# ethz-asl/laser_slam

Hardware: NVIDIA H100
Metric: ICP registrations/s (131072-pt scan vs 524288-pt map, 30 iterations) (higher is better)
Workload: dtype f32

## Files before the change

### laser_slam_b200/csrc/ls_api.cu

```cuda
#include <cerrno>
#include <cmath>
#include <cstdarg>
#include <cstddef>
#include <cstdio>
#include <cstdlib>
#include <cstring>
#include <string>
#include <utility>
#include <vector>

#include "../../include/ls_b200.h"
#include "ls_buffer.cuh"
#include "ls_filters.cuh"
#include "ls_kernels.cuh"
#include "ls_occupancy.cuh"

using namespace ls;

#define LS_VERSION 100

struct Workspace {
  cudaStream_t stream = nullptr;
  cudaEvent_t ev0 = nullptr, ev1 = nullptr, ev2 = nullptr, ev_launch = nullptr;
  Buffer<BuildState> bs;
  Buffer<float4> rd;
  Buffer<int> pos;
  Buffer<float> d2;
  Buffer<float4> vq, vpts;
  Buffer<int> ids;
  Buffer<float> d2_out;
  Buffer<uint32_t> qkey, qperm;
  Buffer<float4> rd_s;
  Buffer<float4> sub_pts, sub_nrm, srt_pts, srt_nrm;
  Buffer<uint32_t> pkey;
  Buffer<Entry> tab1;
  Buffer<uint32_t> cnt1, tab1_cell, qtab_local, qtab_total;
  Buffer<Entry> top;
  Buffer<uint32_t> cnt0;
  Buffer<unsigned long long> pyr, topmask;
  Buffer<uint32_t> qtop_start;
  Buffer<float> T_hist;
  IcpWork* work = nullptr;
  BuildJob* job_host = nullptr;
  BuildJob* job_dev = nullptr;
  IcpProblem hp;
  bool stream_dirty = false;
};

struct ls_ctx {
  int device = 0;
  int sm_count = 0;
  int icp_ctas = 0;
  int icp_ctas_max = 0;
  std::string err;
  uint64_t launches = 0;
  std::vector<Workspace*> ws;
  Buffer<IcpProblem> probs_dev;
  PinnedBuffer<IcpProblem> probs_host;
  Buffer<BuildJob> jobs_dev;
  PinnedBuffer<BuildJob> jobs_host;
  Buffer<IcpWork> work_pool;
  Buffer<IcpResult> results_dev;
  PinnedBuffer<IcpResult> results_host;
  Buffer<float4> reading;
  Buffer<float4> ref_stage, ref_nrm_stage;
  Buffer<float> nrm_raw;
  Buffer<float> T0_dev;
  unsigned char* xbuf = nullptr;
  unsigned char* xpeer[8] = {nullptr, nullptr, nullptr, nullptr, nullptr, nullptr, nullptr, nullptr};
  int shard_rank = 0, shard_count = 1;
  bool xconnected = false;
  unsigned int xflag_base = 0;
  bool pending = false;
  int pending_batch = 0;
  std::vector<int> pending_ws;
  std::vector<int> pending_n;
  std::vector<float> pending_T0;
  std::vector<std::pair<const ls_map*, int>> pending_slots;
  lsf::ChainBuffers chain;
};
constexpr int kMaxBatch = 160;

struct ls_scan_slot {
  Buffer<float4> pts, nrm;
  int n = 0;
  uint64_t id = 0;
  bool used = false;
  cudaEvent_t ready = nullptr;
  bool async = false;
};

constexpr int kStageRing = 16;
struct ls_map {
  ls_ctx* ctx = nullptr;
  int capacity = 0, max_pts = 0;
  uint64_t next_id = 1;
  std::vector<ls_scan_slot> slots;
  cudaStream_t up_stream = nullptr;
  Buffer<float> stage[kStageRing];
  cudaEvent_t stage_free[kStageRing] = {};
  uint64_t n_async = 0;
  PinnedBuffer<float> host_stage[kStageRing];
};

namespace {

int fail(ls_ctx* ctx, int code, const char* fmt, ...) {
  char buf[512];
  va_list ap;
  va_start(ap, fmt);
  vsnprintf(buf, sizeof(buf), fmt, ap);
  va_end(ap);
  if (ctx) ctx->err = buf;
  return code;
}

#define BUSY_CHECK(ctx)                                                                                       \
  do {                                                                                                        \
    if ((ctx)->pending) return fail((ctx), LS_ERR_STATE, "a batch is in flight (ls_icp_register_submap_batch_end first)"); \
  } while (0)

#define CU(call)                                                                                      \
  do {                                                                                                \
    cudaError_t e_ = (call);                                                                          \
    if (e_ != cudaSuccess)                                                                            \
      return fail(ctx, e_ == cudaErrorMemoryAllocation ? LS_ERR_NOMEM : LS_ERR_CUDA, "%s: %s", #call, \
                  cudaGetErrorString(e_));                                                            \
  } while (0)

#define LAUNCH_CHECK()                                                                          \
  do {                                                                                          \
    ++ctx->launches;                                                                            \
    cudaError_t e_ = cudaGetLastError();                                                        \
    if (e_ != cudaSuccess) return fail(ctx, LS_ERR_CUDA, "kernel launch: %s", cudaGetErrorString(e_)); \
  } while (0)

inline int blocks_for(int n, int threads, int cap) {
  int b = (n + threads - 1) / threads;
  if (b < 1) b = 1;
  return b > cap ? cap : b;
}

int grow_failed(ls_ctx* ctx, cudaError_t e, const char* group) {
  return fail(ctx, e == cudaErrorMemoryAllocation ? LS_ERR_NOMEM : LS_ERR_CUDA, "%s: %s", group, cudaGetErrorString(e));
}

int ensure_capacity(ls_ctx* ctx, Workspace* w, int n, int m, int max_cells, int max_iter) {
  cudaError_t e;
  if ((size_t)n > w->rd.capacity()) {
    const size_t c = (size_t)(n + n / 8 + 1024), cv = c * LS_VK;
    if ((e = w->rd.reserve(c, c)) || (e = w->pos.reserve(c, c)) || (e = w->d2.reserve(c, c)) || (e = w->vq.reserve(c, c)) ||
        (e = w->vpts.reserve(cv, cv)) || (e = w->ids.reserve(c, c)) || (e = w->d2_out.reserve(c, c)) ||
        (e = w->qkey.reserve(c, c)) || (e = w->qperm.reserve(c, c)) || (e = w->rd_s.reserve(c, c))) {
      w->rd.reset(), w->pos.reset(), w->d2.reset(), w->vq.reset(), w->vpts.reset(), w->ids.reset(), w->d2_out.reset();
      w->qkey.reset(), w->qperm.reset(), w->rd_s.reset();
      return grow_failed(ctx, e, "reading arrays");
    }
  }
  if ((size_t)m > w->sub_pts.capacity()) {
    const int cap = m + m / 8 + 1024;
    int tcap = cap / 17 + 1024;
    const int tmax = (int)((size_t)1536 * 1024 * 1024 / ((size_t)LS_FB3 * 12));
    if (tcap > tmax) tcap = tmax;
    const size_t c = (size_t)cap, t = (size_t)tcap, tf = t * LS_FB3;
    if ((e = w->sub_pts.reserve(c, c)) || (e = w->sub_nrm.reserve(c, c)) || (e = w->srt_pts.reserve(c, c)) ||
        (e = w->srt_nrm.reserve(c, c)) || (e = w->pkey.reserve(c, c)) || (e = w->tab1.reserve(tf, tf)) ||
        (e = w->cnt1.reserve(tf, tf)) || (e = w->tab1_cell.reserve(t, t)) || (e = w->qtab_local.reserve(tf, tf)) ||
        (e = w->qtab_total.reserve(t, t))) {
      w->sub_pts.reset(), w->sub_nrm.reset(), w->srt_pts.reset(), w->srt_nrm.reset(), w->pkey.reset(), w->tab1.reset();
      w->cnt1.reset(), w->tab1_cell.reset(), w->qtab_local.reset(), w->qtab_total.reset();
      return grow_failed(ctx, e, "sub-map arrays");
    }
    CU(cudaMemsetAsync(w->cnt1.get(), 0, tf * sizeof(uint32_t), w->stream));
    w->stream_dirty = true;
  }
  if ((size_t)max_cells + 1 > w->top.capacity()) {
    const size_t c = (size_t)max_cells + 1, cp = (size_t)max_cells / 2 + 4096;
    if ((e = w->top.reserve(c, c)) || (e = w->cnt0.reserve(c, c)) || (e = w->pyr.reserve(cp, cp)) ||
        (e = w->topmask.reserve(c, c)) || (e = w->qtop_start.reserve(c, c))) {
      w->top.reset(), w->cnt0.reset(), w->pyr.reset(), w->topmask.reset(), w->qtop_start.reset();
      return grow_failed(ctx, e, "cell arrays");
    }
    CU(cudaMemsetAsync(w->cnt0.get(), 0, c * sizeof(uint32_t), w->stream));
    w->stream_dirty = true;
  }
  CU(w->T_hist.reserve((size_t)max_iter * 16, (size_t)max_iter * 16));
  return LS_OK;
}

BuildArrays arrays(const Workspace* w) {
  BuildArrays A;
  A.sub_pts = w->sub_pts.get();
  A.sub_nrm = w->sub_nrm.get();
  A.srt_pts = w->srt_pts.get();
  A.srt_nrm = w->srt_nrm.get();
  A.pkey = w->pkey.get();
  A.top = w->top.get();
  A.cnt0 = w->cnt0.get();
  A.tab1 = w->tab1.get();
  A.cnt1 = w->cnt1.get();
  A.tab1_cell = w->tab1_cell.get();
  A.tab_cap = (int)w->tab1_cell.capacity();
  A.pyr = w->pyr.get();
  A.topmask = w->topmask.get();
  A.qkey = w->qkey.get();
  A.qtop_start = w->qtop_start.get();
  A.qtab_local = w->qtab_local.get();
  A.qtab_total = w->qtab_total.get();
  A.qperm = w->qperm.get();
  A.rd_s = w->rd_s.get();
  return A;
}

int ensure_staging(ls_ctx* ctx, int n, int m) {
  const size_t cn = (size_t)(n + n / 8 + 1024), cm = (size_t)(m + m / 8 + 1024);
  CU(ctx->reading.reserve((size_t)n, cn));
  if ((size_t)m > ctx->ref_stage.capacity()) {
    cudaError_t e;
    if ((e = ctx->ref_stage.reserve(cm, cm)) || (e = ctx->ref_nrm_stage.reserve(cm, cm))) {
      ctx->ref_stage.reset(), ctx->ref_nrm_stage.reset();
      return grow_failed(ctx, e, "reference staging");
    }
  }
  return LS_OK;
}

struct Resolved {
  float cell;
  int split, max_cells;
};

Resolved resolve(const ls_icp_params* p) {
  Resolved r;
  r.cell = p->cell_size > 0.f ? p->cell_size : 1.0f;
  r.split = p->leaf_split > 0 ? (p->leaf_split < 16 ? 16 : p->leaf_split) : 32;
  r.max_cells = p->max_cells > 0 ? p->max_cells : (1 << 22);
  if (r.max_cells > (1 << 22)) r.max_cells = 1 << 22;
  if (r.max_cells < 64) r.max_cells = 64;
// ... 25 lines not shown
  const unsigned int B = (unsigned int)batch;
  const int cap = batch > 1 ? ctx->sm_count * 2 : ctx->sm_count * 8;
  const int pb = blocks_for(m_max, 256, cap);
  reset_build_kernel<<<dim3(1, B), 32, 0, st>>>(jobs_dev);
  LAUNCH_CHECK();
  assemble_kernel<<<dim3(pb, B), 256, 0, st>>>(jobs_dev);
  LAUNCH_CHECK();
  setup_kernel<<<dim3(1, B), 32, 0, st>>>(jobs_dev, r.cell, r.max_cells, r.split);
  LAUNCH_CHECK();
  count0_kernel<<<dim3(pb, B), 256, 0, st>>>(jobs_dev);
  LAUNCH_CHECK();
  const int tiles = (r.max_cells + kScanTile - 1) / kScanTile;
  scan_reduce_kernel<<<dim3(tiles, B), kScanThreads, 0, st>>>(jobs_dev);
  LAUNCH_CHECK();
  scan_apply_kernel<<<dim3(tiles, B), kScanThreads, 0, st>>>(jobs_dev);
  LAUNCH_CHECK();
  pyramid1_kernel<<<dim3(blocks_for(r.max_cells / 16 + 1, 256, batch > 1 ? ctx->sm_count : ctx->sm_count * 4), B), 256, 0, st>>>(jobs_dev);
  LAUNCH_CHECK();
  pyramid_up_kernel<<<dim3(1, B), 1024, 0, st>>>(jobs_dev);
  LAUNCH_CHECK();
  count1_kernel<<<dim3(pb, B), 256, 0, st>>>(jobs_dev);
  LAUNCH_CHECK();
  tables_kernel<<<dim3(cap, B), 256, 0, st>>>(jobs_dev);
  LAUNCH_CHECK();
  scatter_kernel<<<dim3(blocks_for(m_max, 256, ctx->sm_count * 16), B), 256, 0, st>>>(jobs_dev);
  LAUNCH_CHECK();
  return LS_OK;
}

int launch_reading_sort(ls_ctx* ctx, const BuildJob* jobs_dev, int batch, int n_max, const Resolved& r, cudaStream_t st) {
  const unsigned int B = (unsigned int)batch;
  const int cap = batch > 1 ? ctx->sm_count * 2 : ctx->sm_count * 8;
  const int qb = blocks_for(n_max, 256, cap);
  const int scan_tiles = (r.max_cells + kScanTile - 1) / kScanTile;
  q_count_kernel<<<dim3(qb, B), 256, 0, st>>>(jobs_dev);
  LAUNCH_CHECK();
  q_tables_kernel<<<dim3(cap, B), 256, 0, st>>>(jobs_dev);
  LAUNCH_CHECK();
  q_scan_reduce_kernel<<<dim3(scan_tiles, B), kScanThreads, 0, st>>>(jobs_dev);
  LAUNCH_CHECK();
  q_scan_apply_kernel<<<dim3(scan_tiles, B), kScanThreads, 0, st>>>(jobs_dev);
  LAUNCH_CHECK();
  q_scatter_kernel<<<dim3(qb, B), 256, 0, st>>>(jobs_dev);
  LAUNCH_CHECK();
  return LS_OK;
}

int enqueue_build(ls_ctx* ctx, Workspace* w, const Parts& parts, const Resolved& r, const float* T0_host) {
  fill_job(w, parts, T0_host, nullptr, 0);
  CU(cudaMemcpyAsync(w->job_dev, w->job_host, sizeof(BuildJob), cudaMemcpyHostToDevice, w->stream));
  return launch_build(ctx, w->job_dev, 1, w->job_host->m, r, w->stream);
}

int upload_normals(ls_ctx* ctx, Workspace* w, const float* normals, int stride, int n, float4* dst) {
  const size_t need = n > 0 ? (stride <= 8 ? (size_t)(n - 1) * (size_t)stride + 3 : (size_t)n * 3) : 0;
  CU(ctx->nrm_raw.reserve(need, need + 4096));
  int dstride = stride;
  if (stride <= 8) {
    CU(cudaMemcpyAsync(ctx->nrm_raw.get(), normals, need * sizeof(float), cudaMemcpyHostToDevice, w->stream));
  } else {
    CU(cudaMemcpy2DAsync(ctx->nrm_raw.get(), 3 * sizeof(float), normals, (size_t)stride * sizeof(float), 3 * sizeof(float),
                         (size_t)n, cudaMemcpyHostToDevice, w->stream));
    dstride = 3;
  }
  expand_normals_kernel<<<blocks_for(n, 256, ctx->sm_count * 8), 256, 0, w->stream>>>(ctx->nrm_raw.get(), dstride, n, dst);
  LAUNCH_CHECK();
  return LS_OK;
}

int fill_problem(ls_ctx* ctx, Workspace* w, const ls_icp_params* prm, int n, const float T0[16], bool want_matches,
                 bool want_hist) {
  IcpProblem& hp = w->hp;
  hp.bs = w->bs.get();
  hp.view.top = w->top.get();
  hp.view.tab1 = w->tab1.get();
  hp.view.pts = w->srt_pts.get();
  hp.view.pyr = w->pyr.get();
  hp.view.topmask = w->topmask.get();
  hp.nrm = w->srt_nrm.get();
  hp.rd = w->rd_s.get();
  hp.n = n;
  hp.pos = w->pos.get();
  hp.d2 = w->d2.get();
  hp.ids = w->ids.get();
  hp.d2_out = w->d2_out.get();
  hp.qperm = w->qperm.get();
  hp.lists.vq = w->vq.get();
  hp.lists.vpts = w->vpts.get();
  hp.lists.n = n;
  hp.work = w->work;
  hp.shard_rank = 0;
  hp.shard_count = 1;
  std::memset(&hp.link, 0, sizeof(hp.link));
  hp.T_hist = want_hist ? w->T_hist.get() : nullptr;
  if (want_hist) {
    CU(cudaMemsetAsync(w->T_hist.get(), 0, (size_t)prm->max_iterations * 16 * sizeof(float), w->stream));
    w->stream_dirty = true;
  }
  hp.want_matches = want_matches ? 1 : 0;
  hp.phase_ns = nullptr;
  std::memcpy(hp.T0, T0, sizeof(hp.T0));
  return LS_OK;
}

int prep_icp(ls_ctx* ctx, Workspace* w, const ls_icp_params* prm, const float4* reading_dev, int n, const float T0[16],
             bool want_matches, bool want_hist) {
  w->job_host->reading = reading_dev;
  w->job_host->n = n;
  CU(cudaMemcpyAsync(w->job_dev, w->job_host, sizeof(BuildJob), cudaMemcpyHostToDevice, w->stream));
  int rc;
  if ((rc = launch_reading_sort(ctx, w->job_dev, 1, n, resolve(prm), w->stream))) return rc;
  CU(cudaEventRecord(w->ev1, w->stream));
  CU(cudaMemsetAsync(w->work, 0, sizeof(IcpWork), w->stream));
  return fill_problem(ctx, w, prm, n, T0, want_matches, want_hist);
}

int launch_icp(ls_ctx* ctx, const ls_icp_params* prm, int batch, int n_max, bool sharded = false) {
  Workspace* w0 = ctx->ws[0];
  for (int b = 0; b < batch; ++b) ctx->probs_host.get()[b] = ctx->ws[b]->hp;
  CU(cudaMemcpyAsync(ctx->probs_dev.get(), ctx->probs_host.get(), sizeof(IcpProblem) * (size_t)batch, cudaMemcpyHostToDevice,
                     w0->stream));
  IcpParamsDev dp;
  dp.max_iterations = prm->max_iterations;
  dp.trim_ratio = prm->trim_ratio;
  dp.use_differential = prm->use_differential;
  dp.min_diff_rot = prm->min_diff_rot;
  dp.min_diff_trans = prm->min_diff_trans;
  dp.smooth_length = prm->smooth_length;
  int ctas = ctx->icp_ctas / batch;
  const int need = (n_max + 31) / 32;
  if (ctas > need) ctas = need;
  if (ctas < 1) ctas = 1;
  const IcpProblem* probs = ctx->probs_dev.get();
  int dynamic = batch > 1 ? 1 : 0;
  void* args[] = {(void*)&probs, (void*)&ctas, (void*)&dp, (void*)&dynamic};
  if (sharded) {
    shard_slice_kernel<<<1, 32, 0, w0->stream>>>(ctx->probs_dev.get(), w0->job_dev, w0->hp.shard_rank, w0->hp.shard_count);
    LAUNCH_CHECK();
  }
  CU(cudaEventRecord(w0->ev_launch, w0->stream));
  CU(cudaLaunchCooperativeKernel((void*)icp_kernel, dim3(ctas * batch), dim3(kIcpThreads), args, kIcpPairBytes, w0->stream));
  ++ctx->launches;
  CU(cudaEventRecord(w0->ev2, w0->stream));
  collect_results_kernel<<<batch, 32, 0, w0->stream>>>(ctx->probs_dev.get(), ctx->results_dev.get());
  LAUNCH_CHECK();
  CU(cudaMemcpyAsync(ctx->results_host.get(), ctx->results_dev.get(), sizeof(IcpResult) * (size_t)batch, cudaMemcpyDeviceToHost,
                     w0->stream));
  return LS_OK;
}

void launch_times(ls_ctx* ctx, float t[3]) {
  const Workspace* w = ctx->ws[0];
  t[0] = t[1] = t[2] = 0.f;
  cudaEventElapsedTime(&t[0], w->ev0, w->ev2);
  cudaEventElapsedTime(&t[1], w->ev0, w->ev1);
  cudaEventElapsedTime(&t[2], w->ev_launch, w->ev2);
}

int fetch_icp(ls_ctx* ctx, int k, int n, const float T0[16], float T_out[16], ls_icp_stats* stats,
              const float* times = nullptr) {
  const IcpResult& wk = ctx->results_host.get()[k];
  std::memcpy(T_out, wk.T_out, 16 * sizeof(float));
  if (stats) {
    std::memset(stats, 0, sizeof(*stats));
    stats->iterations = wk.iterations;
    stats->converged = wk.converged;
// ... 1578 lines not shown
```

### laser_slam_b200/csrc/ls_kernels.cuh

```cuda
#pragma once
#include <cuda_runtime.h>
#include <cooperative_groups.h>

#include "ls_grid.cuh"

namespace ls {

constexpr int kMaxParts = 16;
constexpr int kScanTile = 4096;
constexpr int kScanThreads = 512;
constexpr int kIcpThreads = 512;
constexpr int kIcpCtasPerSm = 1024 / kIcpThreads;
constexpr int kMaxSmooth = 15;
constexpr uint32_t kTag1 = 1u << 31, kKeyMask = (1u << 31) - 1u;
constexpr int kSubShift = 22;
constexpr uint32_t kCellMask = (1u << kSubShift) - 1u;

struct Parts {
  int n_parts;
  int offset[kMaxParts + 1];
  const float4* pts[kMaxParts];
  const float4* nrm[kMaxParts];
  float T[kMaxParts][16];
  int identity[kMaxParts];
};

struct BuildState {
  unsigned long long sum[3];
  unsigned int minkey[3], maxkey[3];
  Grid grid;
  float T_pre[16];
  unsigned int tile_sums[1024];
};

struct BuildArrays {
  float4* sub_pts;
  float4* sub_nrm;
  float4* srt_pts;
  float4* srt_nrm;
  uint32_t* pkey;
  Entry* top;
  uint32_t* cnt0;
  Entry* tab1;
  uint32_t* cnt1;
  uint32_t* tab1_cell;
  int tab_cap;
  unsigned long long* pyr;
  unsigned long long* topmask;
  uint32_t* qkey;
  uint32_t* qtop_start;
  uint32_t* qtab_local;
  uint32_t* qtab_total;
  uint32_t* qperm;
  float4* rd_s;
};

struct BuildJob {
  Parts parts;
  BuildState* bs;
  BuildArrays A;
  int m;
  int n;
  const float4* reading;
  float4* rd;
  float T0[16];
};

struct IcpParamsDev {
  int max_iterations;
  float trim_ratio;
  int use_differential;
  float min_diff_rot, min_diff_trans;
  int smooth_length;
};

struct alignas(16) IcpWork {
  unsigned int barrier;
  unsigned int pad0[31];
  unsigned int hist[2][5][2048];
  unsigned long long acc[2][32];
  unsigned int qctr[2];
  float T_out[16];
  int status, iterations, converged, max_iter_reached, last_kept;
  float last_limit;
  int fail_code;
  unsigned int xsignals;
  unsigned int dbg_total, dbg_bin[3], dbg_rem[3];
  double dbg_A[6], dbg_x[6];
};

struct IcpResult {
  float T_out[16];
  int status, iterations, converged, max_iter_reached, last_kept;
  float last_limit;
  unsigned int xsignals;
  int n_cells0, n_tab1, overflow;
};

constexpr int kMaxShards = 8;
struct ShardLink {
  IcpWork* slots;
  IcpWork* peer_slots[kMaxShards];
  unsigned int* flag;
  unsigned int* peer_flag[kMaxShards];
  unsigned int flag_base;
};

struct IcpProblem {
  const BuildState* bs;
  GridView view;
  const float4* nrm;
  const float4* rd;
  int n;
  int* pos;
  float* d2;
  int* ids;
  float* d2_out;
  const uint32_t* qperm;
  VLists lists;
  IcpWork* work;
  int shard_rank, shard_count;
  ShardLink link;
  float* T_hist;
  int want_matches;
  unsigned long long* phase_ns;
  float T0[16];
};

__device__ __forceinline__ unsigned int float_order_key(float f) {
  const unsigned int u = __float_as_uint(f);
  return (u & 0x80000000u) ? ~u : (u | 0x80000000u);
}
__device__ __forceinline__ float float_from_order_key(unsigned int k) {
  const unsigned int u = (k & 0x80000000u) ? (k & 0x7fffffffu) : ~k;
  return __uint_as_float(u);
}

__device__ __forceinline__ long long warp_sum_ll(long long v) {
  unsigned int lo = (unsigned int)(v & 0x1FFFFF);
  unsigned int mid = (unsigned int)((v >> 21) & 0x1FFFFF);
  int hi = (int)(v >> 42);
  lo = __reduce_add_sync(0xffffffffu, lo);
  mid = __reduce_add_sync(0xffffffffu, mid);
  hi = __reduce_add_sync(0xffffffffu, hi);
  return ((long long)hi << 42) + ((long long)mid << 21) + (long long)lo;
}

__device__ __forceinline__ void warp_count(uint32_t* ctr, uint32_t key, unsigned int active) {
  const unsigned int peers = __match_any_sync(active, key);
  if ((threadIdx.x & 31) == (unsigned int)(__ffs(peers) - 1)) atomicAdd(ctr, (unsigned int)__popc(peers));
}
__device__ __forceinline__ uint32_t warp_take(uint32_t* ctr, uint32_t key, unsigned int active) {
  const unsigned int peers = __match_any_sync(active, key);
  const int leader = __ffs(peers) - 1;
  const unsigned int lane = threadIdx.x & 31;
  uint32_t old = 0;
  if (lane == (unsigned int)leader) old = atomicSub(ctr, (unsigned int)__popc(peers));
  old = __shfl_sync(peers, old, leader);
  return old - 1u - (uint32_t)__popc(peers & ((1u << lane) - 1u));
}

__global__ void __launch_bounds__(256) assemble_kernel(const BuildJob* __restrict__ jobs) {
  const BuildJob& J = jobs[blockIdx.y];
  const Parts& parts = J.parts;
  float4* __restrict__ sub_pts = J.A.sub_pts;
  float4* __restrict__ sub_nrm = J.A.sub_nrm;
  BuildState* bs = J.bs;
  const int total = parts.offset[parts.n_parts];
  long long s0 = 0, s1 = 0, s2 = 0;
  float mn0 = INFINITY, mn1 = INFINITY, mn2 = INFINITY, mx0 = -INFINITY, mx1 = -INFINITY, mx2 = -INFINITY;
  int p = 0;
  for (int i = blockIdx.x * blockDim.x + threadIdx.x; i < total; i += gridDim.x * blockDim.x) {
    while (i >= parts.offset[p + 1]) ++p;
    const int j = i - parts.offset[p];
    float4 a = __ldg(parts.pts[p] + j);
    float4 nn = __ldg(parts.nrm[p] + j);
    if (!parts.identity[p]) {
      float x, y, z;
      xform_point(parts.T[p], a.x, a.y, a.z, x, y, z);
      a.x = x; a.y = y; a.z = z;
      rotate_vec(parts.T[p], nn.x, nn.y, nn.z, x, y, z);
      nn.x = x; nn.y = y; nn.z = z;
    }
    sub_pts[i] = a;
    sub_nrm[i] = nn;
    s0 += __double2ll_rn((double)a.x * 16777216.0);
    s1 += __double2ll_rn((double)a.y * 16777216.0);
    s2 += __double2ll_rn((double)a.z * 16777216.0);
    mn0 = fminf(mn0, a.x); mx0 = fmaxf(mx0, a.x);
    mn1 = fminf(mn1, a.y); mx1 = fmaxf(mx1, a.y);
    mn2 = fminf(mn2, a.z); mx2 = fmaxf(mx2, a.z);
  }
  s0 = warp_sum_ll(s0); s1 = warp_sum_ll(s1); s2 = warp_sum_ll(s2);
  for (int o = 16; o > 0; o >>= 1) {
    mn0 = fminf(mn0, __shfl_xor_sync(0xffffffffu, mn0, o)); mx0 = fmaxf(mx0, __shfl_xor_sync(0xffffffffu, mx0, o));
    mn1 = fminf(mn1, __shfl_xor_sync(0xffffffffu, mn1, o)); mx1 = fmaxf(mx1, __shfl_xor_sync(0xffffffffu, mx1, o));
    mn2 = fminf(mn2, __shfl_xor_sync(0xffffffffu, mn2, o)); mx2 = fmaxf(mx2, __shfl_xor_sync(0xffffffffu, mx2, o));
  }
// ... 429 lines not shown
  for (int u = threadIdx.x; u < (int)blockIdx.x; u += kScanThreads) s += bs->tile_sums[u];
  s = __reduce_add_sync(0xffffffffu, s);
  if ((threadIdx.x & 31) == 0) ws[threadIdx.x >> 5] = s;
  __syncthreads();
  if (threadIdx.x == 0) {
    unsigned int t = 0;
    for (int w = 0; w < kScanThreads / 32; ++w) t += ws[w];
    tile_off = t;
  }
  __syncthreads();
  constexpr int per = kScanTile / kScanThreads;
  unsigned int c[per], loc = 0;
  const int first = base + threadIdx.x * per;
#pragma unroll
  for (int k = 0; k < per; ++k) {
    c[k] = (first + k < n) ? q_cell_count(A, first + k) : 0u;
    loc += c[k];
  }
  unsigned int incl = loc;
  const int lane = threadIdx.x & 31, warp = threadIdx.x >> 5;
  for (int o = 1; o < 32; o <<= 1) {
    const unsigned int v = __shfl_up_sync(0xffffffffu, incl, o);
    if (lane >= o) incl += v;
  }
  __syncthreads();
  if (lane == 31) ws[warp] = incl;
  __syncthreads();
  unsigned int woff = 0;
  for (int w = 0; w < warp; ++w) woff += ws[w];
  unsigned int run = tile_off + woff + incl - loc;
#pragma unroll
  for (int k = 0; k < per; ++k) {
    if (first + k < n) A.qtop_start[first + k] = run;
    run += c[k];
  }
}

__global__ void __launch_bounds__(256) q_scatter_kernel(const BuildJob* __restrict__ jobs) {
  const BuildArrays A = jobs[blockIdx.y].A;
  const float4* __restrict__ rd = jobs[blockIdx.y].rd;
  const int n = jobs[blockIdx.y].n;
  const int lane = threadIdx.x & 31;
  for (int i = blockIdx.x * blockDim.x + threadIdx.x; i - lane < n; i += gridDim.x * blockDim.x) {
    const unsigned int active = __ballot_sync(0xffffffffu, i < n);
    if (i >= n) break;
    const uint32_t k = A.qkey[i];
    uint32_t start;
    uint32_t* ctr;
    if (k & kTag1) {
      const uint32_t key = k & kKeyMask;
      start = A.qtop_start[A.tab1_cell[key / (uint32_t)LS_FB3]] + A.qtab_local[key];
      ctr = A.cnt1 + key;
    } else {
      start = A.qtop_start[k];
      ctr = A.cnt0 + k;
    }
    const uint32_t rank = start + warp_take(ctr, k, active);
    A.rd_s[rank] = __ldg(rd + i);
    A.qperm[rank] = (uint32_t)i;
  }
}

__global__ void shard_slice_kernel(IcpProblem* P, const BuildJob* __restrict__ job, int shard_rank, int shard_count) {
  if (threadIdx.x != 0 || blockIdx.x != 0) return;
  const BuildArrays A = job->A;
  const int n_cells = job->bs->grid.n_cells0, n = job->n;
  auto cut = [&](int s) -> int {
    if (s <= 0) return 0;
    if (s >= shard_count) return n;
    const unsigned int target = (unsigned int)((long long)n * s / shard_count);
    int lo = 0, hi = n_cells;
    while (lo < hi) {
      const int mid = (lo + hi) >> 1;
      if (A.qtop_start[mid] < target) lo = mid + 1;
      else hi = mid;
    }
    return lo < n_cells ? (int)A.qtop_start[lo] : n;
  };
  const int q0 = cut(shard_rank), q1 = cut(shard_rank + 1);
  P->rd += q0;
  P->qperm += q0;
  P->pos += q0;
  P->d2 += q0;
  P->lists.vq += q0;
  P->lists.vpts += q0;
  P->n = q1 - q0;
}

__global__ void collect_results_kernel(const IcpProblem* __restrict__ probs, IcpResult* __restrict__ out) {
  const IcpProblem& P = probs[blockIdx.x];
  const IcpWork* W = P.work;
  IcpResult& r = out[blockIdx.x];
  if (threadIdx.x < 16) r.T_out[threadIdx.x] = W->T_out[threadIdx.x];
  if (threadIdx.x == 0) {
    r.status = W->status;
    r.iterations = W->iterations;
    r.converged = W->converged;
    r.max_iter_reached = W->max_iter_reached;
    r.last_kept = W->last_kept;
    r.last_limit = W->last_limit;
    r.xsignals = W->xsignals;
    r.n_cells0 = P.bs->grid.n_cells0;
    r.n_tab1 = P.bs->grid.n_tab1;
    r.overflow = P.bs->grid.overflow;
  }
}

__global__ void __launch_bounds__(256) reading_kernel(const BuildJob* __restrict__ jobs) {
  const BuildState* __restrict__ bs = jobs[blockIdx.y].bs;
  const float4* __restrict__ in = jobs[blockIdx.y].reading;
  float4* __restrict__ out = jobs[blockIdx.y].rd;
  const int n = jobs[blockIdx.y].n;
  __shared__ float T[16];
  if (threadIdx.x < 16) T[threadIdx.x] = bs->T_pre[threadIdx.x];
  __syncthreads();
  for (int i = blockIdx.x * blockDim.x + threadIdx.x; i < n; i += gridDim.x * blockDim.x) {
    const float4 a = __ldg(in + i);
    float4 o;
    xform_point(T, a.x, a.y, a.z, o.x, o.y, o.z);
    o.w = a.w;
    out[i] = o;
  }
}

__global__ void __launch_bounds__(256) transform_kernel(const float* __restrict__ Tg, const float4* __restrict__ in,
                                                        const float4* __restrict__ nin, int n, float4* __restrict__ out,
                                                        float4* __restrict__ nout) {
  __shared__ float T[16];
  if (threadIdx.x < 16) T[threadIdx.x] = Tg[threadIdx.x];
  __syncthreads();
  for (int i = blockIdx.x * blockDim.x + threadIdx.x; i < n; i += gridDim.x * blockDim.x) {
    const float4 a = __ldg(in + i);
    float4 o;
    xform_point(T, a.x, a.y, a.z, o.x, o.y, o.z);
    o.w = a.w;
    out[i] = o;
    if (nin) {
      const float4 b = __ldg(nin + i);
      float4 r;
      rotate_vec(T, b.x, b.y, b.z, r.x, r.y, r.z);
      r.w = 0.f;
      nout[i] = r;
    }
  }
}

__global__ void pack_normals_kernel(const float4* __restrict__ in, int n, float* __restrict__ out3) {
  for (int i = blockIdx.x * blockDim.x + threadIdx.x; i < n; i += gridDim.x * blockDim.x) {
    const float4 a = in[i];
    out3[3 * (size_t)i] = a.x;
    out3[3 * (size_t)i + 1] = a.y;
    out3[3 * (size_t)i + 2] = a.z;
  }
}

__global__ void __launch_bounds__(256) nn_query_kernel(const BuildState* __restrict__ bs, GridView view,
                                                       const float4* __restrict__ rd, int n, int* __restrict__ ids,
                                                       float* __restrict__ d2) {
  __shared__ Grid g;
  if (threadIdx.x == 0) g = bs->grid;
  __syncthreads();
  for (int i = blockIdx.x * blockDim.x + threadIdx.x; i < n; i += gridDim.x * blockDim.x) {
    const float4 q = __ldg(rd + i);
    const Best b = nn_search(g, view, q.x, q.y, q.z, -1, INFINITY);
    ids[i] = b.idx;
    d2[i] = b.d2;
// ... 181 lines not shown
  }
  if (first) {
    k = (unsigned int)((float)total * ratio);
    if (total > 0 && k >= total) k = total - 1;
  }
  unsigned int run = woff + incl - loc;
  for (int j = 0; j < per; ++j) {
    if (k >= run && k < run + c[j]) {
      out->bin = threadIdx.x * per + j;
      out->rem = k - run;
    }
    run += c[j];
  }
  if (threadIdx.x == 0) out->total = total;
  __syncthreads();
}


struct SelHists {
  unsigned int h1[1024];
  unsigned int h2[2048];
  unsigned int h3[1024];
};
constexpr unsigned int kNoPrediction = 0xffffffffu;

__device__ __forceinline__ void phase_a_record(const IcpProblem& P, int i, const Best& b, SelHists* H, unsigned int pred_bin1,
                                               unsigned int pred_pref12) {
  if (b.pos >= 0) __stcg(P.pos + i, b.pos);
  const float d = b.pos >= 0 ? b.d2 : INFINITY;
  __stcg(P.d2 + i, d);
  const unsigned int key = __float_as_uint(d);
  if (key <= 0x7f800000u) {
    atomicAdd(&H->h1[key >> 21], 1u);
    if ((key >> 21) == pred_bin1) {
      atomicAdd(&H->h2[(key >> 10) & 2047u], 1u);
      if ((key >> 10) == pred_pref12) atomicAdd(&H->h3[key & 1023u], 1u);
    }
  }
}

__device__ __forceinline__ void residual_terms(float sx, float sy, float sz, const float4 q, const float4 nn, float* f, float& e) {
  float u = sy * nn.z, v = sz * nn.y;
  f[0] = u - v;
  u = sz * nn.x; v = sx * nn.z;
  f[1] = u - v;
  u = sx * nn.y; v = sy * nn.x;
  f[2] = u - v;
  f[3] = nn.x; f[4] = nn.y; f[5] = nn.z;
  const float dx = sx - q.x, dy = sy - q.y, dz = sz - q.z;
  e = dx * nn.x;
  float t = dy * nn.y;
  e = e + t;
  t = dz * nn.z;
  e = e + t;
}

constexpr int kPairSlots = 64;
constexpr int kIcpPairBytes = (kIcpThreads / 32) * kPairSlots * 8 * (int)sizeof(float);
__constant__ unsigned char kPairRow[32] = {0, 0, 0, 0, 0, 0, 1, 1, 1, 1, 1, 2, 2, 2, 2, 3, 3, 3, 4, 4, 5, 0, 1, 2, 3, 4, 5, 7, 7, 7, 7, 7};
__constant__ unsigned char kPairCol[32] = {0, 1, 2, 3, 4, 5, 1, 2, 3, 4, 5, 2, 3, 4, 5, 3, 4, 5, 4, 5, 5, 6, 6, 6, 6, 6, 6, 7, 7, 7, 7, 7};

struct PairQueue {
  float* recs;
  int head, cnt;
  long long acc;
};

__device__ __noinline__ long long consume_pairs(const float* recs, int head, int count, long long acc) {
  const int lane = threadIdx.x & 31;
  const int ro = kPairRow[lane], co = kPairCol[lane];
  const float scale = lane < 27 ? 4194304.0f : 1.0f;
#pragma unroll 4
  for (int j = 0; j < count; ++j) {
    const float* r = recs + ((head + j) & (kPairSlots - 1)) * 8;
    const float a = r[ro], b = r[co], sg = r[7];
    long long v = __float2ll_rn((a * b) * scale);
    if (sg < 0.f) v = -v;
    acc += v;
  }
  return acc;
}

__device__ __forceinline__ void push_pairs(const IcpProblem& P, PairQueue& Q, int sign, float sx, float sy, float sz,
                                           const float4 q, int pos) {
  const unsigned int m = __ballot_sync(0xffffffffu, sign != 0);
  if (m == 0u) return;
  if (sign) {
    float f[6], e;
    residual_terms(sx, sy, sz, q, __ldg(P.nrm + pos), f, e);
    const int slot = (Q.head + Q.cnt + __popc(m & ((1u << (threadIdx.x & 31)) - 1u))) & (kPairSlots - 1);
    float4* r = reinterpret_cast<float4*>(Q.recs + slot * 8);
    r[0] = make_float4(f[0], f[1], f[2], f[3]);
    r[1] = make_float4(f[4], f[5], e, (float)sign);
  }
  Q.cnt += __popc(m);
  __syncwarp();
  if (Q.cnt >= 32) {
    Q.acc = consume_pairs(Q.recs, Q.head, 32, Q.acc);
    Q.head = (Q.head + 32) & (kPairSlots - 1);
    Q.cnt -= 32;
    __syncwarp();
  }
}

__device__ __forceinline__ void drain_pairs(PairQueue& Q, unsigned long long* slab) {
  if (Q.cnt > 0) {
    Q.acc = consume_pairs(Q.recs, Q.head, Q.cnt, Q.acc);
    Q.head = (Q.head + Q.cnt) & (kPairSlots - 1);
    Q.cnt = 0;
  }
  const int lane = threadIdx.x & 31;
  if (lane < 28) slab[lane] = (unsigned long long)Q.acc;
  Q.acc = 0ll;
  __syncwarp();
}

__device__ __noinline__ void phase_a_search(const Grid* gp, const IcpProblem* Pp, const float* T_iter, const float* T_prev,
                                            int i, float cap, SelHists* H, unsigned int pred_bin1, unsigned int pred_pref12) {
  if (i < 0) return;
  const Grid& g = *gp;
  const IcpProblem& P = *Pp;
  const float4 r = __ldg(P.rd + i);
  float sx, sy, sz;
  xform_point(T_iter, r.x, r.y, r.z, sx, sy, sz);
  const int warm = __ldcg(P.pos + i);
  const Best b = nn_search(g, P.view, sx, sy, sz, warm, cap);
  phase_a_record(P, i, b, H, pred_bin1, pred_pref12);
  if (T_prev) {
    float px, py, pz;
    xform_point(T_prev, r.x, r.y, r.z, px, py, pz);
    vlist_build(g, P.view, P.lists, i, sx, sy, sz, b.pos >= 0, b.d2, cap, sqrtf(dist2(sx, sy, sz, px, py, pz)));
  }
}

__device__ __forceinline__ void push_searched(const IcpProblem& P, PairQueue& Q, const float* T_iter, int j, float acc_limit) {
  if (!(acc_limit >= 0.0f)) return;
  float d = INFINITY;
  if (j >= 0) d = __ldcg(P.d2 + j);
  const bool keep = d <= acc_limit;
  if (__ballot_sync(0xffffffffu, keep) == 0u) return;
  float4 q = make_float4(0.f, 0.f, 0.f, 0.f);
  float sx = 0.f, sy = 0.f, sz = 0.f;
  int pos = -1;
  if (keep) {
    pos = __ldcg(P.pos + j);
    const float4 r = __ldg(P.rd + j);
    xform_point(T_iter, r.x, r.y, r.z, sx, sy, sz);
    q = __ldg(P.view.pts + pos);
  }
  push_pairs(P, Q, keep ? 1 : 0, sx, sy, sz, q, pos);
}

__device__ __noinline__ void final_match(const Grid* gp, const IcpProblem* Pp, const float* T, int i) {
  if (i < 0) return;
  const IcpProblem& P = *Pp;
  const float4 r = __ldg(P.rd + i);
  float sx, sy, sz;
  xform_point(T, r.x, r.y, r.z, sx, sy, sz);
  const Best b = nn_search(*gp, P.view, sx, sy, sz, __ldcg(P.pos + i), INFINITY);
  const uint32_t orig = __ldg(P.qperm + i);
  P.d2_out[orig] = b.d2;
  P.ids[orig] = b.idx;
}

__device__ __forceinline__ void flush_slabs(unsigned long long (*acc_w)[28], unsigned long long* gacc) {
  __syncthreads();
  if (threadIdx.x < 28) {
    unsigned long long t = 0ull;
#pragma unroll
    for (int w = 0; w < kIcpThreads / 32; ++w) t += acc_w[w][threadIdx.x];
    if (t != 0ull) atomicAdd(&gacc[threadIdx.x], t);
  }
  __syncthreads();
}

__device__ __forceinline__ void flush_hist(const unsigned int* hs, int nbins, unsigned int* gh) {
  for (int k = threadIdx.x; k < nbins; k += kIcpThreads) {
    const unsigned int v = hs[k];
    if (v) atomicAdd(&gh[k], v);
  }
}

__global__ void __launch_bounds__(kIcpThreads, kIcpCtasPerSm)
icp_kernel(const IcpProblem* __restrict__ probs, int ctas_per_problem, IcpParamsDev prm, int dynamic) {
  const int pi = blockIdx.x / ctas_per_problem;
  const int cta = blockIdx.x - pi * ctas_per_problem;
  const IcpProblem& P = probs[pi];
  IcpWork* W = P.work;
  const bool xg = P.shard_count > 1;
  IcpWork* X = xg ? P.link.slots + P.shard_rank : W;
  const IcpWork* S0 = xg ? P.link.slots : W;
  const int n_slots = xg ? P.shard_count : 1;
  const unsigned int G = (unsigned int)ctas_per_problem;
  unsigned int xepoch = 0;
  const int tid = threadIdx.x, lane = tid & 31;

  __shared__ Grid g;
  __shared__ float T_iter[16], T_last[16];
  __shared__ SelHists hs;
  __shared__ unsigned long long acc_w[kIcpThreads / 32][28];
  __shared__ SelectOut sel;
  __shared__ unsigned int ws[kIcpThreads / 32];
  __shared__ double qh[kMaxSmooth + 2][4];
  __shared__ double th[kMaxSmooth + 2][3];
  __shared__ int flag_stop, flag_status;
  __shared__ int miss_buf[kIcpThreads / 32][64];
  extern __shared__ __align__(16) float pair_buf[];

  if (tid == 0) {
    g = P.bs->grid;
    for (int i = 0; i < 16; ++i) T_iter[i] = (i % 5 == 0) ? 1.f : 0.f;
    quat_from_T(T_iter, qh[0]);
    th[0][0] = th[0][1] = th[0][2] = 0.0;
    flag_stop = 0;
    flag_status = 0;
  }
  __syncthreads();
  PairQueue Q;
  Q.recs = pair_buf + (tid >> 5) * (kPairSlots * 8);
  Q.head = 0;
  Q.cnt = 0;
  Q.acc = 0ll;

  const int n = P.n;
  int chunk = (n + (int)G - 1) / (int)G;
  chunk = (chunk + 31) & ~31;
  const int q_begin = min(n, cta * chunk), q_end = min(n, q_begin + chunk);

  for (int i = q_begin + tid; i < q_end; i += kIcpThreads) {
    __stcg(P.pos + i, -1);
    __stcg(P.lists.vq + i, make_float4(0.f, 0.f, 0.f, 0.f));
  }

  float cap = 0.04f;
  int redo = 0;
  unsigned int epoch = 0;
  constexpr int kHistOff = (int)(offsetof(IcpWork, hist) / 4), kAccOff = (int)(offsetof(IcpWork, acc) / 4);
  auto meet = [&](int off0, int n0, int off1, int n1, int off2, int n2) {
    if (xg) shard_exchange(P, X, cta, G, epoch, xepoch, off0, n0, off1, n1, off2, n2);
    else problem_barrier(&X->barrier, G, epoch);
  };
  problem_barrier(&X->barrier, G, epoch);
  int hist_count = 1;
  int iter = 0, converged = 0, max_reached = 0, last_kept = 0;
  float last_limit = 0.f;
  unsigned int pred_bin1 = kNoPrediction, pred_pref12 = kNoPrediction;
  float acc_limit = -1.0f;

  for (;;) {
    const int par = iter & 1;
    LS_STAMP(0);
    for (int k = tid; k < (int)(sizeof(SelHists) / 4); k += kIcpThreads) reinterpret_cast<unsigned int*>(&hs)[k] = 0u;
    __syncthreads();
    {
      const float* T_prev = iter >= 1 ? T_last : nullptr;
      int* mq = miss_buf[tid >> 5];
      int n_miss = 0;
      int next = q_begin + (tid & ~31);
      for (;;) {
        int base;
        if (dynamic) {
          unsigned int bb = 0;
          if (lane == 0) bb = atomicAdd(&W->qctr[par], 32u);
          bb = __shfl_sync(0xffffffffu, bb, 0);
          if (bb >= (unsigned int)n) break;
          base = (int)bb;
        } else {
          if (next >= q_end) break;
          base = next;
          next += kIcpThreads;
        }
        const int i = base + lane;
        bool valid = i < (dynamic ? n : q_end);
        if (redo && valid) valid = !(__ldcg(P.d2 + i) < INFINITY);
        bool hit = false;
        Best b;
        b.d2 = INFINITY; b.idx = INT_MAX; b.pos = -1;
        float4 c = make_float4(0.f, 0.f, 0.f, 0.f);
        float sx = 0.f, sy = 0.f, sz = 0.f;
        if (valid) {
          const float4 r = __ldg(P.rd + i);
          const float4 v = __ldcg(P.lists.vq + i);
          const float4 c0 = __ldcg(P.lists.vpts + i);
          xform_point(T_iter, r.x, r.y, r.z, sx, sy, sz);
          hit = vlist_query(P.lists, P.view.pts, i, v, c0, sx, sy, sz, cap, b, c);
          if (hit) phase_a_record(P, i, b, &hs, pred_bin1, pred_pref12);
        }
        push_pairs(P, Q, (hit && b.pos >= 0 && b.d2 <= acc_limit) ? 1 : 0, sx, sy, sz, c, b.pos);
        const unsigned int mm = __ballot_sync(0xffffffffu, valid && !hit);
        if (mm) {
          if (valid && !hit) mq[n_miss + __popc(mm & ((1u << lane) - 1u))] = i;
          n_miss += __popc(mm);
          __syncwarp();
          if (n_miss >= 32) {
            n_miss -= 32;
            const int j = mq[n_miss + lane];
            __syncwarp();
            phase_a_search(&g, &P, T_iter, T_prev, j, cap, &hs, pred_bin1, pred_pref12);
            push_searched(P, Q, T_iter, j, acc_limit);
          }
        }
      }
      if (n_miss > 0) {
        __syncwarp();
        const int j = lane < n_miss ? mq[lane] : -1;
        phase_a_search(&g, &P, T_iter, T_prev, j, cap, &hs, pred_bin1, pred_pref12);
        __syncwarp();
        push_searched(P, Q, T_iter, j, acc_limit);
      }
    }
    drain_pairs(Q, acc_w[tid >> 5]);
    flush_slabs(acc_w, X->acc[par]);
    flush_hist(hs.h1, 1024, X->hist[par][0]);
    if (pred_bin1 != kNoPrediction) {
      flush_hist(hs.h2, 2048, X->hist[par][3]);
      flush_hist(hs.h3, 1024, X->hist[par][4]);
    }
    {
      const int hb = kHistOff + par * 5 * 2048;
      const bool pr = pred_bin1 != kNoPrediction;
      meet(hb, 1024, hb + 3 * 2048, pr ? 2048 : 0, hb + 4 * 2048, pr ? 1024 : 0);
    }
    LS_STAMP(1);

    block_select(S0->hist[par][0], 1024, 0u, true, prm.trim_ratio, &sel, ws, n_slots);
    if (sel.total == 0u) {
      if (tid == 0) { flag_status = 1; if (cta == 0) W->fail_code = 1; }
      __syncthreads();
      break;
    }
    if (sel.bin >= 1020u) {
      if (!(cap < INFINITY)) {
        if (tid == 0) { flag_status = 1; if (cta == 0) W->fail_code = 1; }
        __syncthreads();
        break;
      }
      cap = cap < 64.0f ? cap * 4.0f : INFINITY;
      ++redo;
      meet(0, 0, 0, 0, 0, 0);
      if (cta == 0 && tid == 0) {
        X->hist[par][0][1020] = 0u;
        W->qctr[par] = 0u;
      }
      problem_barrier(&X->barrier, G, epoch);
      continue;
    }
    const unsigned int bin1 = sel.bin, rem1 = sel.rem;
    if (cta == 0) {
      unsigned int* h = &X->hist[par ^ 1][0][0];
      for (int k = tid; k < 5 * 2048; k += kIcpThreads) h[k] = 0u;
      if (tid < 32) X->acc[par ^ 1][tid] = 0ull;
    }
    if (cta == 0 && tid == 0) W->qctr[par ^ 1] = 0u;
    const bool spec2 = bin1 == pred_bin1;
    if (!spec2) {
      for (int k = tid; k < 2048; k += kIcpThreads) hs.h2[k] = 0u;
      __syncthreads();
      for (int i = q_begin + tid; i < q_end; i += kIcpThreads) {
        const unsigned int key = __float_as_uint(__ldcg(P.d2 + i));
        if (key < 0x7f800000u && (key >> 21) == bin1) atomicAdd(&hs.h2[(key >> 10) & 2047u], 1u);
      }
      __syncthreads();
      flush_hist(hs.h2, 2048, X->hist[par][1]);
      meet(kHistOff + (par * 5 + 1) * 2048, 2048, 0, 0, 0, 0);
    }
    LS_STAMP(2);
    block_select(S0->hist[par][spec2 ? 3 : 1], 2048, rem1, false, 0.f, &sel, ws, n_slots);
    const unsigned int bin2 = sel.bin, rem2 = sel.rem;
    const unsigned int prefix12 = (bin1 << 11) | bin2;
    const bool spec3 = spec2 && prefix12 == pred_pref12;
    if (!spec3) {
      for (int k = tid; k < 1024; k += kIcpThreads) hs.h3[k] = 0u;
      __syncthreads();
      for (int i = q_begin + tid; i < q_end; i += kIcpThreads) {
        const unsigned int key = __float_as_uint(__ldcg(P.d2 + i));
        if (key < 0x7f800000u && (key >> 10) == prefix12) atomicAdd(&hs.h3[key & 1023u], 1u);
      }
      __syncthreads();
      flush_hist(hs.h3, 1024, X->hist[par][2]);
      meet(kHistOff + (par * 5 + 2) * 2048, 1024, 0, 0, 0, 0);
    }
    LS_STAMP(3);
    block_select(S0->hist[par][spec3 ? 4 : 2], 1024, rem2, false, 0.f, &sel, ws, n_slots);
    const float limit = __uint_as_float((prefix12 << 10) | sel.bin);
    cap = fmaxf(limit * (iter == 0 ? 0.5f : 2.0f), 1e-12f);
    redo = 0;

    for (int base = q_begin; base < q_end; base += kIcpThreads) {
      const int i = base + tid;
      int sign = 0, pos = -1;
      if (i < q_end) {
        const float d = __ldcg(P.d2 + i);
        pos = __ldcg(P.pos + i);
        sign = ((d <= limit && pos >= 0) ? 1 : 0) - ((d <= acc_limit) ? 1 : 0);
      }
      if (__ballot_sync(0xffffffffu, sign != 0) == 0u) continue;
      float sx = 0.f, sy = 0.f, sz = 0.f;
      float4 q = make_float4(0.f, 0.f, 0.f, 0.f);
      if (sign) {
        const float4 r = __ldg(P.rd + i);
        xform_point(T_iter, r.x, r.y, r.z, sx, sy, sz);
        q = __ldg(P.view.pts + pos);
      }
      push_pairs(P, Q, sign, sx, sy, sz, q, pos);
    }
    drain_pairs(Q, acc_w[tid >> 5]);
    flush_slabs(acc_w, X->acc[par]);
    meet(kAccOff + par * 64, 64, 0, 0, 0, 0);
    LS_STAMP(4);

    if (tid == 0) {
      double A[36], b[6], x[6];
      int k = 0;
      for (int rr = 0; rr < 6; ++rr)
        for (int cc = rr; cc < 6; ++cc, ++k) {
          const double v = (double)(long long)sum_slots_u64(&S0->acc[par][k], n_slots) / 4194304.0;
          A[rr * 6 + cc] = v;
          A[cc * 6 + rr] = v;
        }
      for (int rr = 0; rr < 6; ++rr) b[rr] = -((double)(long long)sum_slots_u64(&S0->acc[par][21 + rr], n_slots) / 4194304.0);
      last_kept = (int)sum_slots_u64(&S0->acc[par][27], n_slots);
      last_limit = limit;
      int status = 0, stop = 0;
      if (last_kept == 0) {
        status = 1;
        if (cta == 0) W->fail_code = 2;
      } else {
        if (!chol6(A, b, x)) jacobi_pinv_solve6(A, b, x);
        for (int i = 0; i < 6; ++i)
          if (!is_finite_d(x[i])) status = 1;
        if (status && cta == 0) W->fail_code = 3;
      }
      if (cta == 0) {
        W->dbg_total = sel.total; W->dbg_bin[0] = bin1; W->dbg_bin[1] = bin2; W->dbg_bin[2] = sel.bin;
        W->dbg_rem[0] = rem1; W->dbg_rem[1] = rem2; W->dbg_rem[2] = sel.rem;
        for (int i = 0; i < 6; ++i) { W->dbg_A[i] = A[i * 6 + i]; W->dbg_x[i] = x[i]; }
      }
      if (!status) {
        float T_step[16];
        step_matrix(x, T_step);
        for (int i = 0; i < 16; ++i) T_last[i] = T_iter[i];
        mat4_mul(T_step, T_iter, T_iter);
        if (P.T_hist && cta == 0)
          for (int i = 0; i < 16; ++i) P.T_hist[iter * 16 + i] = T_iter[i];
        if (iter + 1 >= prm.max_iterations) { stop = 1; max_reached = 1; }
        if (prm.use_differential) {
          const int L = prm.smooth_length;
          if (hist_count == L + 1) {
            for (int i = 0; i < L; ++i) {
              for (int c = 0; c < 4; ++c) qh[i][c] = qh[i + 1][c];
              for (int c = 0; c < 3; ++c) th[i][c] = th[i + 1][c];
            }
            --hist_count;
          }
          quat_from_T(T_iter, qh[hist_count]);
          th[hist_count][0] = (double)T_iter[12];
          th[hist_count][1] = (double)T_iter[13];
          th[hist_count][2] = (double)T_iter[14];
          ++hist_count;
          if (hist_count > L) {
            double mr = 0.0, mt = 0.0;
            for (int i = hist_count - 1; i >= hist_count - L; --i) {
              mr += fabs(quat_angular_distance(qh[i], qh[i - 1]));
              const double ddx = th[i][0] - th[i - 1][0], ddy = th[i][1] - th[i - 1][1], ddz = th[i][2] - th[i - 1][2];
              mt += sqrt(ddx * ddx + ddy * ddy + ddz * ddz);
            }
            mr /= (double)L;
            mt /= (double)L;
            if (mr != mr || mt != mt) { status = 1; if (cta == 0) W->fail_code = 4; }
            else if (mr < (double)prm.min_diff_rot && mt < (double)prm.min_diff_trans) { stop = 1; converged = 1; }
          }
        }
      }
      flag_status = status;
      flag_stop = stop | status;
      LS_STAMP(5);
    }
    __syncthreads();
    if (!flag_status) ++iter;
    if (flag_stop) break;
    pred_bin1 = bin1;
    pred_pref12 = prefix12;
    acc_limit = iter >= 2 ? limit : -1.0f;
  }

  if (P.want_matches && !flag_status && iter > 0) {
    for (int base = q_begin; base < q_end; base += kIcpThreads) final_match(&g, &P, T_last, base + tid < q_end ? base + tid : -1);
// ... 24 lines not shown
```

Baseline: 976.3.

## Restrict correction pass to boundary-bin list and cache matched normals per point

During phase A each CTA appends the indices of points whose distance falls in the predicted trim bin to a global boundary list. When the speculated bin is confirmed, the correction pass walks only that list instead of scanning every query. A per-point cache of the matched normal, tagged with its map index, avoids reloading normals when the match has not changed, and the IcpProblem struct is copied into shared memory. This adds global atomics, extra buffers and extra stores in the hot loop, and falls back to the full scan when the list overflows.

```diff
diff --git a/laser_slam_b200/csrc/ls_api.cu b/laser_slam_b200/csrc/ls_api.cu
--- a/laser_slam_b200/csrc/ls_api.cu
+++ b/laser_slam_b200/csrc/ls_api.cu
@@ -26,6 +26,8 @@
   Buffer<float4> rd;
   Buffer<int> pos;
   Buffer<float> d2;
+  Buffer<float4> mn;
+  Buffer<int> blist;
   Buffer<float4> vq, vpts;
   Buffer<int> ids;
   Buffer<float> d2_out;
@@ -148,12 +150,13 @@
 int ensure_capacity(ls_ctx* ctx, Workspace* w, int n, int m, int max_cells, int max_iter) {
   cudaError_t e;
   if ((size_t)n > w->rd.capacity()) {
-    const size_t c = (size_t)(n + n / 8 + 1024), cv = c * LS_VK;
-    if ((e = w->rd.reserve(c, c)) || (e = w->pos.reserve(c, c)) || (e = w->d2.reserve(c, c)) || (e = w->vq.reserve(c, c)) ||
-        (e = w->vpts.reserve(cv, cv)) || (e = w->ids.reserve(c, c)) || (e = w->d2_out.reserve(c, c)) ||
-        (e = w->qkey.reserve(c, c)) || (e = w->qperm.reserve(c, c)) || (e = w->rd_s.reserve(c, c))) {
-      w->rd.reset(), w->pos.reset(), w->d2.reset(), w->vq.reset(), w->vpts.reset(), w->ids.reset(), w->d2_out.reset();
-      w->qkey.reset(), w->qperm.reset(), w->rd_s.reset();
+    const size_t c = (size_t)(n + n / 8 + 1024), cv = c * LS_VK, cb = 2 * (size_t)blist_cap((int)c);
+    if ((e = w->rd.reserve(c, c)) || (e = w->pos.reserve(c, c)) || (e = w->d2.reserve(c, c)) || (e = w->mn.reserve(c, c)) ||
+        (e = w->blist.reserve(cb, cb)) || (e = w->vq.reserve(c, c)) || (e = w->vpts.reserve(cv, cv)) ||
+        (e = w->ids.reserve(c, c)) || (e = w->d2_out.reserve(c, c)) || (e = w->qkey.reserve(c, c)) ||
+        (e = w->qperm.reserve(c, c)) || (e = w->rd_s.reserve(c, c))) {
+      w->rd.reset(), w->pos.reset(), w->d2.reset(), w->mn.reset(), w->blist.reset(), w->vq.reset(), w->vpts.reset();
+      w->ids.reset(), w->d2_out.reset(), w->qkey.reset(), w->qperm.reset(), w->rd_s.reset();
       return grow_failed(ctx, e, "reading arrays");
     }
   }
@@ -345,6 +348,8 @@
   hp.n = n;
   hp.pos = w->pos.get();
   hp.d2 = w->d2.get();
+  hp.mn = w->mn.get();
+  hp.blist = w->blist.get();
   hp.ids = w->ids.get();
   hp.d2_out = w->d2_out.get();
   hp.qperm = w->qperm.get();
diff --git a/laser_slam_b200/csrc/ls_kernels.cuh b/laser_slam_b200/csrc/ls_kernels.cuh
--- a/laser_slam_b200/csrc/ls_kernels.cuh
+++ b/laser_slam_b200/csrc/ls_kernels.cuh
@@ -80,6 +80,7 @@
   unsigned int hist[2][5][2048];
   unsigned long long acc[2][32];
   unsigned int qctr[2];
+  unsigned int bctr[2];
   float T_out[16];
   int status, iterations, converged, max_iter_reached, last_kept;
   float last_limit;
@@ -114,6 +115,8 @@
   int n;
   int* pos;
   float* d2;
+  float4* mn;
+  int* blist;
   int* ids;
   float* d2_out;
   const uint32_t* qperm;
@@ -709,6 +712,7 @@
   P->qperm += q0;
   P->pos += q0;
   P->d2 += q0;
+  P->mn += q0;
   P->lists.vq += q0;
   P->lists.vpts += q0;
   P->n = q1 - q0;
@@ -1056,12 +1060,18 @@
 }
 
 __device__ __forceinline__ void push_pairs(const IcpProblem& P, PairQueue& Q, int sign, float sx, float sy, float sz,
-                                           const float4 q, int pos) {
+                                           const float4 q, int pos, int i, const float4 mn) {
   const unsigned int m = __ballot_sync(0xffffffffu, sign != 0);
   if (m == 0u) return;
   if (sign) {
+    float4 nn = mn;
+    if (f2i(mn.w) != pos) {
+      nn = __ldg(P.nrm + pos);
+      nn.w = i2f(pos);
+      __stcg(P.mn + i, nn);
+    }
     float f[6], e;
-    residual_terms(sx, sy, sz, q, __ldg(P.nrm + pos), f, e);
+    residual_terms(sx, sy, sz, q, nn, f, e);
     const int slot = (Q.head + Q.cnt + __popc(m & ((1u << (threadIdx.x & 31)) - 1u))) & (kPairSlots - 1);
     float4* r = reinterpret_cast<float4*>(Q.recs + slot * 8);
     r[0] = make_float4(f[0], f[1], f[2], f[3]);
@@ -1107,22 +1117,43 @@
   }
 }
 
-__device__ __forceinline__ void push_searched(const IcpProblem& P, PairQueue& Q, const float* T_iter, int j, float acc_limit) {
+struct BoundaryList {
+  unsigned int* ctr;
+  int* ranks;
+  unsigned int cap;
+};
+__host__ __device__ __forceinline__ unsigned int blist_cap(int n) { return (unsigned int)(n / 16 + 256); }
+
+__device__ __forceinline__ void blist_append(const BoundaryList& L, bool in, int i) {
+  const unsigned int m = __ballot_sync(0xffffffffu, in);
+  if (m == 0u) return;
+  const int lane = threadIdx.x & 31;
+  unsigned int base = 0u;
+  if (lane == 0) base = atomicAdd(L.ctr, (unsigned int)__popc(m));
+  base = __shfl_sync(0xffffffffu, base, 0);
+  const unsigned int k = base + (unsigned int)__popc(m & ((1u << lane) - 1u));
+  if (in && k < L.cap) __stcg(L.ranks + k, i);
+}
+
+__device__ __forceinline__ void push_searched(const IcpProblem& P, PairQueue& Q, const BoundaryList& L, const float* T_iter,
+                                              int j, float acc_limit, unsigned int pred_bin1) {
   if (!(acc_limit >= 0.0f)) return;
   float d = INFINITY;
   if (j >= 0) d = __ldcg(P.d2 + j);
+  blist_append(L, d < INFINITY && (__float_as_uint(d) >> 21) == pred_bin1, j);
   const bool keep = d <= acc_limit;
   if (__ballot_sync(0xffffffffu, keep) == 0u) return;
-  float4 q = make_float4(0.f, 0.f, 0.f, 0.f);
+  float4 q = make_float4(0.f, 0.f, 0.f, 0.f), mn = q;
   float sx = 0.f, sy = 0.f, sz = 0.f;
   int pos = -1;
   if (keep) {
     pos = __ldcg(P.pos + j);
+    mn = __ldcg(P.mn + j);
     const float4 r = __ldg(P.rd + j);
     xform_point(T_iter, r.x, r.y, r.z, sx, sy, sz);
     q = __ldg(P.view.pts + pos);
   }
-  push_pairs(P, Q, keep ? 1 : 0, sx, sy, sz, q, pos);
+  push_pairs(P, Q, keep ? 1 : 0, sx, sy, sz, q, pos, j, mn);
 }
 
 __device__ __noinline__ void final_match(const Grid* gp, const IcpProblem* Pp, const float* T, int i) {
@@ -1159,7 +1190,12 @@
 icp_kernel(const IcpProblem* __restrict__ probs, int ctas_per_problem, IcpParamsDev prm, int dynamic) {
   const int pi = blockIdx.x / ctas_per_problem;
   const int cta = blockIdx.x - pi * ctas_per_problem;
-  const IcpProblem& P = probs[pi];
+  __shared__ IcpProblem Ps;
+  static_assert(sizeof(IcpProblem) % 4 == 0, "copied as 32-bit words");
+  for (int k = threadIdx.x; k < (int)(sizeof(IcpProblem) / 4); k += kIcpThreads)
+    reinterpret_cast<unsigned int*>(&Ps)[k] = reinterpret_cast<const unsigned int*>(probs + pi)[k];
+  __syncthreads();
+  const IcpProblem& P = Ps;
   IcpWork* W = P.work;
   const bool xg = P.shard_count > 1;
   IcpWork* X = xg ? P.link.slots + P.shard_rank : W;
@@ -1203,8 +1239,10 @@
 
   for (int i = q_begin + tid; i < q_end; i += kIcpThreads) {
     __stcg(P.pos + i, -1);
+    __stcg(P.mn + i, make_float4(0.f, 0.f, 0.f, i2f(-1)));
     __stcg(P.lists.vq + i, make_float4(0.f, 0.f, 0.f, 0.f));
   }
+  const unsigned int bcap = blist_cap(n);
 
   float cap = 0.04f;
   int redo = 0;
@@ -1223,6 +1261,7 @@
 
   for (;;) {
     const int par = iter & 1;
+    const BoundaryList L{&W->bctr[par], P.blist + par * bcap, bcap};
     LS_STAMP(0);
     for (int k = tid; k < (int)(sizeof(SelHists) / 4); k += kIcpThreads) reinterpret_cast<unsigned int*>(&hs)[k] = 0u;
     __syncthreads();
@@ -1250,17 +1289,19 @@
         bool hit = false;
         Best b;
         b.d2 = INFINITY; b.idx = INT_MAX; b.pos = -1;
-        float4 c = make_float4(0.f, 0.f, 0.f, 0.f);
+        float4 c = make_float4(0.f, 0.f, 0.f, 0.f), mn = c;
         float sx = 0.f, sy = 0.f, sz = 0.f;
         if (valid) {
           const float4 r = __ldg(P.rd + i);
           const float4 v = __ldcg(P.lists.vq + i);
           const float4 c0 = __ldcg(P.lists.vpts + i);
+          if (acc_limit >= 0.0f) mn = __ldcg(P.mn + i);
           xform_point(T_iter, r.x, r.y, r.z, sx, sy, sz);
           hit = vlist_query(P.lists, P.view.pts, i, v, c0, sx, sy, sz, cap, b, c);
           if (hit) phase_a_record(P, i, b, &hs, pred_bin1, pred_pref12);
         }
-        push_pairs(P, Q, (hit && b.pos >= 0 && b.d2 <= acc_limit) ? 1 : 0, sx, sy, sz, c, b.pos);
+        push_pairs(P, Q, (hit && b.pos >= 0 && b.d2 <= acc_limit) ? 1 : 0, sx, sy, sz, c, b.pos, i, mn);
+        if (acc_limit >= 0.0f) blist_append(L, hit && b.pos >= 0 && (__float_as_uint(b.d2) >> 21) == pred_bin1, i);
         const unsigned int mm = __ballot_sync(0xffffffffu, valid && !hit);
         if (mm) {
           if (valid && !hit) mq[n_miss + __popc(mm & ((1u << lane) - 1u))] = i;
@@ -1271,7 +1312,7 @@
             const int j = mq[n_miss + lane];
             __syncwarp();
             phase_a_search(&g, &P, T_iter, T_prev, j, cap, &hs, pred_bin1, pred_pref12);
-            push_searched(P, Q, T_iter, j, acc_limit);
+            push_searched(P, Q, L, T_iter, j, acc_limit, pred_bin1);
           }
         }
       }
@@ -1280,7 +1321,7 @@
         const int j = lane < n_miss ? mq[lane] : -1;
         phase_a_search(&g, &P, T_iter, T_prev, j, cap, &hs, pred_bin1, pred_pref12);
         __syncwarp();
-        push_searched(P, Q, T_iter, j, acc_limit);
+        push_searched(P, Q, L, T_iter, j, acc_limit, pred_bin1);
       }
     }
     drain_pairs(Q, acc_w[tid >> 5]);
@@ -1325,7 +1366,7 @@
       for (int k = tid; k < 5 * 2048; k += kIcpThreads) h[k] = 0u;
       if (tid < 32) X->acc[par ^ 1][tid] = 0ull;
     }
-    if (cta == 0 && tid == 0) W->qctr[par ^ 1] = 0u;
+    if (cta == 0 && tid == 0) W->qctr[par ^ 1] = W->bctr[par ^ 1] = 0u;
     const bool spec2 = bin1 == pred_bin1;
     if (!spec2) {
       for (int k = tid; k < 2048; k += kIcpThreads) hs.h2[k] = 0u;
@@ -1360,23 +1401,30 @@
     cap = fmaxf(limit * (iter == 0 ? 0.5f : 2.0f), 1e-12f);
     redo = 0;
 
-    for (int base = q_begin; base < q_end; base += kIcpThreads) {
-      const int i = base + tid;
+    const unsigned int bcnt = (spec2 && acc_limit >= 0.0f) ? __ldcg(L.ctr) : 0xffffffffu;
+    const bool from_list = bcnt <= bcap;
+    const int c_begin = from_list ? cta * kIcpThreads : q_begin;
+    const int c_end = from_list ? (int)bcnt : q_end;
+    const int c_step = from_list ? (int)G * kIcpThreads : kIcpThreads;
+    for (int base = c_begin; base < c_end; base += c_step) {
+      int i = base + tid;
       int sign = 0, pos = -1;
-      if (i < q_end) {
+      if (i < c_end) {
+        if (from_list) i = __ldcg(L.ranks + i);
         const float d = __ldcg(P.d2 + i);
         pos = __ldcg(P.pos + i);
         sign = ((d <= limit && pos >= 0) ? 1 : 0) - ((d <= acc_limit) ? 1 : 0);
       }
       if (__ballot_sync(0xffffffffu, sign != 0) == 0u) continue;
       float sx = 0.f, sy = 0.f, sz = 0.f;
-      float4 q = make_float4(0.f, 0.f, 0.f, 0.f);
+      float4 q = make_float4(0.f, 0.f, 0.f, 0.f), mn = q;
       if (sign) {
         const float4 r = __ldg(P.rd + i);
         xform_point(T_iter, r.x, r.y, r.z, sx, sy, sz);
         q = __ldg(P.view.pts + pos);
+        mn = __ldcg(P.mn + i);
       }
-      push_pairs(P, Q, sign, sx, sy, sz, q, pos);
+      push_pairs(P, Q, sign, sx, sy, sz, q, pos, i, mn);
     }
     drain_pairs(Q, acc_w[tid >> 5]);
     flush_slabs(acc_w, X->acc[par]);
```

New measurement: 976.7 (median of 6 runs). No clear change (+0.0%).
